# MDFahimAnjum/AliasFree-Diffusion-Models-PyTorch

Hardware: AMD Instinct MI355X
Metric: train_step_images_per_sec (higher is better)
Workload: dtype f32; 1 GPU; CIFAR-10 32x32x3 synthetic, UNet variant=3 (Config D), batch 256/GPU, T=1000, AdamW lr 3e-4, random-init weights (seed 42); global_batch=256, parallelism=dp1, hip_graph=True, launch_mode=lanes

## Files before the change

aliasfree-diffusion-models-pytorch_amd/_lib.py:

```python
import ctypes
import os
import re

_PKG = os.path.dirname(os.path.abspath(__file__))
_ROOT = os.path.dirname(_PKG)
HEADER = os.path.join(_ROOT, "include", "afd.h")
LIBPATH = os.environ.get("AFD_LIBPATH") or os.path.join(_PKG, "libafd_hip.so")

_CTYPES = {
    "int": ctypes.c_int, "long": ctypes.c_long, "float": ctypes.c_float, "double": ctypes.c_double,
    "size_t": ctypes.c_size_t,
}
_DECL = re.compile(r"^(int|size_t|const char\*)\s+(afd_\w+)\s*\(([^;]*?)\)\s*;", re.M | re.S)


def _strip_comments(src):
    return re.sub(r"/\*.*?\*/", " ", src, flags=re.S)


def parse_header(path=HEADER):
    out = {}
    for ret, name, args in _DECL.findall(_strip_comments(open(path).read())):
        argtypes = []
        args = " ".join(args.split())
        if args not in ("", "void"):
            for a in args.split(","):
                a = a.strip()
                if "*" in a or a.startswith("afd_stream_t"):
                    argtypes.append(ctypes.c_void_p)
                else:
                    base = a.split()[0] if not a.startswith("unsigned") else a
                    argtypes.append(_CTYPES[base])
        restype = {"int": ctypes.c_int, "size_t": ctypes.c_size_t, "const char*": ctypes.c_char_p}[ret]
        out[name] = (restype, argtypes)
    return out


_VALUE_RETURNING = {"afd_device_count", "afd_tok_supported", "afd_conv3x3_weight_kinds", "afd_conv_wgrad_form",
                    "afd_grad_sqnorm_n_partials"}


class AfdError(RuntimeError):
    pass


class _Lib:
    def __init__(self):
        if not os.path.exists(LIBPATH):
            raise AfdError(
                f"{LIBPATH} not found: build it with `python -c 'import __graft_entry__ as g; g.build()'` "
                "(hipcc --offload-arch=gfx950). There is no CPU/eager fallback.")
        self.cdll = ctypes.CDLL(LIBPATH)
        self.sigs = parse_header()
        for name, (restype, argtypes) in self.sigs.items():
            fn = getattr(self.cdll, name)
            fn.restype, fn.argtypes = restype, argtypes
            if restype is ctypes.c_int and name not in _VALUE_RETURNING:
                setattr(self, name, self._checked(name, fn))
            else:
                setattr(self, name, fn)

    def _checked(self, name, fn):
        last_error = self.cdll.afd_last_error
        last_error.restype = ctypes.c_char_p

        def call(*args):
            rc = fn(*args)
            if rc != 0:
                raise AfdError(f"{name} failed (code {rc}): {last_error().decode()}")
        call.__name__ = name
        return call


_lib = None


def lib():
    global _lib
    if _lib is None:
        _lib = _Lib()
    return _lib
```

aliasfree-diffusion-models-pytorch_amd/csrc/filt.hip:

```cpp
#include "common.h"

namespace afd {

__global__ void up2_fwd_gen(const float* __restrict__ x, float* __restrict__ y, int C, int H, int W,
                            long xbs, long ybs, long total, Taps t, int N) {
  const int lo = (N - 1) / 2, H2 = 2 * H, W2 = 2 * W;
  for (long i = blockIdx.x * (long)blockDim.x + threadIdx.x; i < total; i += (long)gridDim.x * blockDim.x) {
    const int q = i % W2, p = (i / W2) % H2;
    const long bc = i / ((long)W2 * H2);
    const int c = bc % C; const long b = bc / C;
    const float* xp = x + b * xbs + (long)c * H * W;
    float acc = 0.f;
    for (int a = 0; a < N; ++a) {
      const int zr = p + a - lo;
      if (zr < 0 || zr >= H2 || (zr & 1)) continue;
      for (int bb = 0; bb < N; ++bb) {
        const int zc = q + bb - lo;
        if (zc < 0 || zc >= W2 || (zc & 1)) continue;
        acc += t.k[a * N + bb] * xp[(zr >> 1) * W + (zc >> 1)];
      }
    }
    y[b * ybs + (long)c * H2 * W2 + (long)p * W2 + q] = acc;
  }
}
// ... 171 lines not shown
  xv[S] = 0.f;
  float2* yp = reinterpret_cast<float2*>(y + b * ybs + (long)c * 4 * S * S) + L.col;
  float xr = L.right(xv[0]);
#pragma unroll
  for (int i = 0; i < S; ++i) {
    const float xe = xv[i], xd = xv[i + 1];
    const float xdr = L.right(xd);
    float2 r0, r1;
    r0.x = t.k[4] * xe;
    r0.y = t.k[3] * xe + t.k[5] * xr;
    r1.x = t.k[1] * xe + t.k[7] * xd;
    r1.y = t.k[0] * xe + t.k[2] * xr + t.k[6] * xd + t.k[8] * xdr;
    if (live) { yp[(2 * i) * S] = r0; yp[(2 * i + 1) * S] = r1; }
    xr = xdr;
  }
}

template <int S, bool FULL>
__global__ __launch_bounds__(256) void down2_fwd_n3(const float* __restrict__ x, float* __restrict__ y,
                                                    long planes, int C, long xbs, long ybs, Taps3 t) {
  Lane<S> L(planes);
  if (FULL && !L.live) return;
  const bool live = FULL || L.live;
  const long b = L.plane / C; const int c = L.plane % C;
  const float2* xp = reinterpret_cast<const float2*>(x + b * xbs + (long)c * 4 * S * S) + L.col;
  float* yp = y + b * ybs + (long)c * S * S + L.col;
  float2 prev = make_float2(0.f, 0.f);
  float prev_l = 0.f;
  float2 rows[2 * S];
#pragma unroll
  for (int r = 0; r < 2 * S; ++r) rows[r] = live ? xp[r * S] : make_float2(0.f, 0.f);
#pragma unroll
  for (int i = 0; i < S; ++i) {
    const float2 mid = rows[2 * i], nxt = rows[2 * i + 1];
    const float mid_l = L.left(mid.y), nxt_l = L.left(nxt.y);
    const float d = t.k[0] * prev_l + t.k[1] * prev.x + t.k[2] * prev.y
                  + t.k[3] * mid_l  + t.k[4] * mid.x  + t.k[5] * mid.y
                  + t.k[6] * nxt_l  + t.k[7] * nxt.x  + t.k[8] * nxt.y;
    if (live) yp[i * S] = d;
    prev = nxt; prev_l = nxt_l;
  }
}

struct ActRow { float U[4], t[4]; float4 c[4]; };
struct ActG { float g00, g01, g10, g11, g01l, g11l; };

__device__ __forceinline__ void act_lookup(float U, const float4* __restrict__ T, float& t, float4& c) {
  const float sx = __builtin_amdgcn_fmed3f(fmaf(U, kGeluScale, kGeluOffset), 0.f, (float)kGeluPieces - 0.001f);
  c = T[(int)sx];
  t = __builtin_amdgcn_fractf(sx);
}
__device__ __forceinline__ float act_cubic(const float4& c, float t) { return fmaf(fmaf(fmaf(c.w, t, c.z), t, c.y), t, c.x); }

template <int S, bool FULL, bool STATS = false>
__global__ __launch_bounds__(STATS ? 1024 : 256) void filt_act_fwd_n3(const float* __restrict__ x, float* __restrict__ y,
                                                       long planes, int C, const float* __restrict__ stats,
                                                       const float* __restrict__ gamma, const float* __restrict__ beta,
                                                       const float* __restrict__ res, Taps3 u, Taps3 d,
                                                       float* __restrict__ stats_out = nullptr, float eps = 0.f) {
  __shared__ float4 T[kGeluPieces];
  load_gelu_table(T, 0, kGeluPieces);
  Lane<S> L(planes);
  const long b = L.plane / C; const int c = L.plane % C;
  const long base = L.plane * (long)S * S + L.col;
  if (FULL && !L.live) return;
  const bool live = FULL || L.live;
  float sc, sh;
  float xv[S + 2];
  if (STATS) {
    __shared__ float red[16];
#pragma unroll
    for (int i = 0; i < S; ++i) xv[i] = x[base + i * S];
    float sm = 0.f;
#pragma unroll
    for (int i = 0; i < S; ++i) sm += xv[i];
    const float n = (float)C * S * S;
    const float mean = block_sum(sm, red) / n;
    float m2 = 0.f;
#pragma unroll
    for (int i = 0; i < S; ++i) { const float dd = xv[i] - mean; m2 = fmaf(dd, dd, m2); }
    const float rstd = 1.0f / sqrtf(block_sum(m2, red) / n + eps);
    if (threadIdx.x == 0) { stats_out[2 * b] = mean; stats_out[2 * b + 1] = rstd; }
    sc = rstd * (gamma ? gamma[c] : 1.f);
    sh = (beta ? beta[c] : 0.f) - mean * sc;
#pragma unroll
    for (int i = 0; i < S; ++i) xv[i] = fmaf(xv[i], sc, sh);
  } else {
    if (live) plane_affine(stats, gamma, beta, b, c, sc, sh); else { sc = 1.f; sh = 0.f; }
#pragma unroll
    for (int i = 0; i < S; ++i) xv[i] = live ? fmaf(x[base + i * S], sc, sh) : 0.f;
  }
  if (res) {
#pragma unroll
    for (int i = 0; i < S; ++i) xv[i] += live ? res[base + i * S] : 0.f;
  }
  xv[S] = 0.f; xv[S + 1] = 0.f;
  ActRow row[2];
  ActG gg[2];
  float g10p = 0.f, g11p = 0.f, g11lp = 0.f;
  float xr0 = L.right(xv[0]), xr1 = lane_right(xv[1]);
#pragma unroll
  for (int k = 0; k < S + 2; ++k) {
    if (k < S) {
      ActRow& r = row[k & 1];
      const float xe = xv[k], xd = xv[k + 1];
      xr1 = L.right_mask(xr1);
      r.U[0] = u.k[4] * xe;
      r.U[1] = u.k[3] * xe + u.k[5] * xr0;
      r.U[2] = u.k[1] * xe + u.k[7] * xd;
      r.U[3] = u.k[0] * xe + u.k[2] * xr0 + u.k[6] * xd + u.k[8] * xr1;
#pragma unroll
      for (int q = 0; q < 4; ++q) act_lookup(r.U[q], T, r.t[q], r.c[q]);
      xr0 = xr1;
      xr1 = (k + 2 <= S) ? lane_right(xv[k + 2]) : 0.f;
    }
    __builtin_amdgcn_sched_barrier(0);
    if (k >= 2) {
      const ActG& g = gg[k & 1];
      const float g01l = L.left_mask(g.g01l), g11l = L.left_mask(g.g11l);
      const float out = d.k[0] * g11lp + d.k[1] * g10p + d.k[2] * g11p
                      + d.k[3] * g01l + d.k[4] * g.g00 + d.k[5] * g.g01
                      + d.k[6] * g11l + d.k[7] * g.g10 + d.k[8] * g.g11;
      if (live) y[base + (k - 2) * S] = out;
      g10p = g.g10; g11p = g.g11; g11lp = g11l;
    }
    __builtin_amdgcn_sched_barrier(0);
    if (k >= 1 && k <= S) {
      const ActRow& r = row[(k - 1) & 1];
      ActG& g = gg[(k - 1) & 1];
      g.g00 = r.U[0] * act_cubic(r.c[0], r.t[0]);
      g.g01 = r.U[1] * act_cubic(r.c[1], r.t[1]);
      g.g10 = r.U[2] * act_cubic(r.c[2], r.t[2]);
      g.g11 = r.U[3] * act_cubic(r.c[3], r.t[3]);
      g.g01l = lane_left(g.g01);
      g.g11l = lane_left(g.g11);
    }
    __builtin_amdgcn_sched_barrier(0);
  }
}

struct ActRowB { float t[4], dG[4]; float4 c[4]; };
struct ActGB { float dU00, dU01, dU10, dU11, dU01l, dU11l; };

template <int S, bool FULL, bool GNB = false>
__global__ __launch_bounds__(GNB ? 1024 : 256) void filt_act_bwd_n3(const float* __restrict__ x, const float* __restrict__ dy,
                                                       float* __restrict__ dv, long planes, int C,
                                                       const float* __restrict__ stats, const float* __restrict__ gamma,
                                                       const float* __restrict__ beta, const float* __restrict__ res,
                                                       float* __restrict__ part, Taps3 u, Taps3 d, float* __restrict__ dx = nullptr) {
  __shared__ float4 Tb[kGeluPieces];
  load_gelu_table(Tb, kGeluPieces, kGeluPieces);
  Lane<S> L(planes);
  const long b = L.plane / C; const int c = L.plane % C;
  const long base = L.plane * (long)S * S + L.col;
  if (FULL && !L.live) return;
  const bool live = FULL || L.live;
  float sc, sh;
  if (live) plane_affine(stats, gamma, beta, b, c, sc, sh); else { sc = 1.f; sh = 0.f; }
  float mean = 0.f, rstd = 1.f;
  if (part && live) { mean = stats[2 * b]; rstd = stats[2 * b + 1]; }
  float xv[S + 2], gv[S + 2];
  float a1 = 0.f, a2 = 0.f;
  float hx[S];
  float dvc[GNB ? S : 1];
#pragma unroll
  for (int i = 0; i < S; ++i) {
    const float h = live ? x[base + i * S] : 0.f;
    xv[i] = live ? fmaf(h, sc, sh) : 0.f;
    hx[i] = (h - mean) * rstd;
    gv[i] = live ? dy[base + i * S] : 0.f;
  }
  if (res) {
#pragma unroll
    for (int i = 0; i < S; ++i) xv[i] += live ? res[base + i * S] : 0.f;
  }
  xv[S] = 0.f; gv[S] = 0.f; xv[S + 1] = 0.f; gv[S + 1] = 0.f;
  ActRowB row[2];
  ActGB gg[2];
  float u10p = 0.f, u11p = 0.f, u11lp = 0.f;
  float xr0 = L.right(xv[0]), xr1 = lane_right(xv[1]), gr0 = L.right(gv[0]), gr1 = lane_right(gv[1]);
#pragma unroll
  for (int k = 0; k < S + 2; ++k) {
    if (k < S) {
      ActRowB& r = row[k & 1];
      const float xe = xv[k], xd = xv[k + 1], ge = gv[k], gd = gv[k + 1];
      xr1 = L.right_mask(xr1); gr1 = L.right_mask(gr1);
      const float U00 = u.k[4] * xe;
      const float U01 = u.k[3] * xe + u.k[5] * xr0;
      const float U10 = u.k[1] * xe + u.k[7] * xd;
      const float U11 = u.k[0] * xe + u.k[2] * xr0 + u.k[6] * xd + u.k[8] * xr1;
      act_lookup(U00, Tb, r.t[0], r.c[0]);
      act_lookup(U01, Tb, r.t[1], r.c[1]);
      act_lookup(U10, Tb, r.t[2], r.c[2]);
      act_lookup(U11, Tb, r.t[3], r.c[3]);
      r.dG[0] = d.k[4] * ge;
      r.dG[1] = d.k[5] * ge + d.k[3] * gr0;
      r.dG[2] = d.k[7] * ge + d.k[1] * gd;
      r.dG[3] = d.k[8] * ge + d.k[6] * gr0 + d.k[2] * gd + d.k[0] * gr1;
      xr0 = xr1; gr0 = gr1;
      xr1 = (k + 2 <= S) ? lane_right(xv[k + 2]) : 0.f;
      gr1 = (k + 2 <= S) ? lane_right(gv[k + 2]) : 0.f;
    }
    __builtin_amdgcn_sched_barrier(0);
    if (k >= 2) {
      const ActGB& g = gg[k & 1];
      const float dU01l = L.left_mask(g.dU01l), dU11l = L.left_mask(g.dU11l);
      const float out = u.k[0] * g.dU11 + u.k[1] * g.dU10 + u.k[2] * dU11l
                      + u.k[3] * g.dU01 + u.k[4] * g.dU00 + u.k[5] * dU01l
                      + u.k[6] * u11p + u.k[7] * u10p + u.k[8] * u11lp;
      if (GNB) { dvc[k - 2] = out; if (dv) dv[base + (k - 2) * S] = out; }
      else if (live) dv[base + (k - 2) * S] = out;
      a1 += out * hx[k - 2]; a2 += out;
      u10p = g.dU10; u11p = g.dU11; u11lp = dU11l;
    }
    __builtin_amdgcn_sched_barrier(0);
    if (k >= 1 && k <= S) {
      const ActRowB& r = row[(k - 1) & 1];
      ActGB& g = gg[(k - 1) & 1];
      g.dU00 = r.dG[0] * act_cubic(r.c[0], r.t[0]);
      g.dU01 = r.dG[1] * act_cubic(r.c[1], r.t[1]);
      g.dU10 = r.dG[2] * act_cubic(r.c[2], r.t[2]);
      g.dU11 = r.dG[3] * act_cubic(r.c[3], r.t[3]);
      g.dU01l = lane_left(g.dU01);
      g.dU11l = lane_left(g.dU11);
    }
    __builtin_amdgcn_sched_barrier(0);
  }
  if (GNB) {
    __shared__ float red[16];
    const float g = gamma ? gamma[c] : 1.f, n = (float)C * S * S;
    const float m1 = block_sum(g * a2, red) / n;
    const float m2 = block_sum(g * a1, red) / n;
#pragma unroll
    for (int i = 0; i < S; ++i) dx[base + i * S] = rstd * (g * dvc[i] - m1 - hx[i] * m2);
  }
  if (part) {
#pragma unroll
    for (int o = S / 2; o > 0; o >>= 1) { a1 += __shfl_xor(a1, o, kWave); a2 += __shfl_xor(a2, o, kWave); }
    if (live && L.col == 0) { part[(2 * b) * C + c] = a1; part[(2 * b + 1) * C + c] = a2; }
  }
}

static inline int gs_grid(long total, int block = 256) {
  long g = (total + block - 1) / block;
  return (int)(g < 1 ? 1 : (g > 65536 ? 65536 : g));
}
static inline bool fast_side(int H, int W) { return H == W && (H == 4 || H == 8 || H == 16 || H == 32 || H == 64); }
static inline Taps load_taps(const float* k, int N) { Taps t; for (int i = 0; i < N * N; ++i) t.k[i] = k[i]; return t; }
static inline Taps3 load_taps3(const float* k, bool rot180 = false) {
  Taps3 t; for (int i = 0; i < 9; ++i) t.k[i] = k[rot180 ? 8 - i : i]; return t;
}


#define AFD_DISPATCH_SF(S_, KERNEL, GRID_ARGS, ...)                                                      \
  if (planes % (64 / (S_)) == 0) hipLaunchKernelGGL((KERNEL<S_, true>), GRID_ARGS, __VA_ARGS__);          \
  else hipLaunchKernelGGL((KERNEL<S_, false>), GRID_ARGS, __VA_ARGS__)
#define AFD_DISPATCH_S(S_, KERNEL, GRID_ARGS, ...)                                          \
  switch (S_) {                                                                              \
    case 4:  AFD_DISPATCH_SF(4, KERNEL, GRID_ARGS, __VA_ARGS__); break;                      \
    case 8:  AFD_DISPATCH_SF(8, KERNEL, GRID_ARGS, __VA_ARGS__); break;                      \
    case 16: AFD_DISPATCH_SF(16, KERNEL, GRID_ARGS, __VA_ARGS__); break;                     \
    case 32: AFD_DISPATCH_SF(32, KERNEL, GRID_ARGS, __VA_ARGS__); break;                     \
    default: AFD_DISPATCH_SF(64, KERNEL, GRID_ARGS, __VA_ARGS__); break;                     \
  }

static inline dim3 fast_grid(long planes, int S) {
  const long ppw = 64 / S, waves = (planes + ppw - 1) / ppw;
  return dim3((unsigned)((waves + 3) / 4));
}

static int check_common(const char* fn, const void* a, const void* b, int B, int C, int H, int W, const float* taps, int N) {
  AFD_REQUIRE(a && b && taps, "%s: NULL pointer", fn);
  AFD_REQUIRE(B > 0 && C > 0 && H > 0 && W > 0, "%s: non-positive shape B=%d C=%d H=%d W=%d", fn, B, C, H, W);
  AFD_REQUIRE(N >= 1 && N <= AFD_MAX_TAPS, "%s: N=%d outside [1,%d]", fn, N, AFD_MAX_TAPS);
  return AFD_OK;
}

static int up2_like(const char* fn, const float* x, float* y, int B, int C, int H, int W, long xbs, long ybs,
                    const float* taps, int N, bool rot, hipStream_t s) {
  if (!xbs) xbs = (long)C * H * W;
  if (!ybs) ybs = (long)C * 4 * H * W;
  const long planes = (long)B * C;
  if (N == 3 && fast_side(H, W)) {
    const Taps3 t = load_taps3(taps, rot);
    AFD_DISPATCH_S(H, up2_fwd_n3, fast_grid(planes, H), dim3(256), 0, s, x, y, planes, C, xbs, ybs, t);
  } else {
    AFD_REQUIRE(!rot, "%s: internal: rot180 only on the fast path", fn);
    const long total = planes * 4 * H * W;
    hipLaunchKernelGGL(up2_fwd_gen, dim3(gs_grid(total)), dim3(256), 0, s, x, y, C, H, W, xbs, ybs, total, load_taps(taps, N), N);
  }
  return check_launch(fn);
}
// ... 40 lines not shown
  return check_launch("afd_filt_up2_bwd");
}

int afd_filt_down2_fwd(const float* x, float* y, int B, int C, int H, int W, long xbs, long ybs,
                       const float* taps, int N, afd_stream_t stream) {
  if (int e = check_common("afd_filt_down2_fwd", x, y, B, C, H, W, taps, N)) return e;
  return down2_like("afd_filt_down2_fwd", x, y, B, C, H, W, xbs, ybs, taps, N, false, as_stream(stream));
}

int afd_filt_down2_bwd(const float* dy, float* dx, int B, int C, int H, int W, long dybs, long dxbs,
                       const float* taps, int N, afd_stream_t stream) {
  if (int e = check_common("afd_filt_down2_bwd", dy, dx, B, C, H, W, taps, N)) return e;
  hipStream_t s = as_stream(stream);
  const int Ho = (H + 1) / 2, Wo = (W + 1) / 2;
  if (N == 3 && (H % 2 == 0) && (W % 2 == 0) && fast_side(Ho, Wo))
    return up2_like("afd_filt_down2_bwd", dy, dx, B, C, Ho, Wo, dybs, dxbs, taps, N, true, s);
  if (!dybs) dybs = (long)C * Ho * Wo;
  if (!dxbs) dxbs = (long)C * H * W;
  const long total = (long)B * C * H * W;
  hipLaunchKernelGGL(down2_bwd_gen, dim3(gs_grid(total)), dim3(256), 0, s, dy, dx, C, H, W, dybs, dxbs, total, load_taps(taps, N), N);
  return check_launch("afd_filt_down2_bwd");
}

size_t afd_filt_act_workspace_bytes(int B, int C, int H, int W, int N, int backward) {
  if (N == 3 && fast_side(H, W)) return 0;
  const size_t e = (size_t)B * C * H * W;
  return sizeof(float) * (backward ? 9 * e : 5 * e);
}

int afd_filt_act_fwd(const float* x, float* y, int B, int C, int H, int W,
                     const float* stats, const float* gamma, const float* beta, const float* res,
                     const float* taps_up, const float* taps_down, int N, void* workspace, afd_stream_t stream) {
  if (int e = check_common("afd_filt_act_fwd", x, y, B, C, H, W, taps_up, N)) return e;
  AFD_REQUIRE(taps_down, "afd_filt_act_fwd: taps_down is NULL");
  hipStream_t s = as_stream(stream);
  const long planes = (long)B * C;
  if (N == 3 && fast_side(H, W)) {
    const Taps3 u = load_taps3(taps_up), d = load_taps3(taps_down);
    ensure_gelu_table(s);
    AFD_DISPATCH_S(H, filt_act_fwd_n3, fast_grid(planes, H), dim3(256), 0, s, x, y, planes, C, stats, gamma, beta, res, u, d);
    return check_launch("afd_filt_act_fwd");
  }
  AFD_REQUIRE(workspace, "afd_filt_act_fwd: this shape (N=%d, %dx%d) needs a workspace", N, H, W);
  const long e = planes * H * W;
  float* v = static_cast<float*>(workspace);
  float* U = v + e;
  hipLaunchKernelGGL(prologue_gen, dim3(gs_grid(e)), dim3(256), 0, s, x, v, C, (long)H * W, e, stats, gamma, beta, res);
  hipLaunchKernelGGL(up2_fwd_gen, dim3(gs_grid(4 * e)), dim3(256), 0, s, v, U, C, H, W, (long)C * H * W, (long)C * 4 * H * W, 4 * e, load_taps(taps_up, N), N);
  hipLaunchKernelGGL(gelu_inplace_gen, dim3(gs_grid(4 * e)), dim3(256), 0, s, U, 4 * e);
  hipLaunchKernelGGL(down2_fwd_gen, dim3(gs_grid(e)), dim3(256), 0, s, U, y, C, 2 * H, 2 * W, (long)C * 4 * H * W, (long)C * H * W, e, load_taps(taps_down, N), N);
  return check_launch("afd_filt_act_fwd");
}

size_t afd_filt_act_fwd_gn_supported(int C, int H, int W, int N) {
  return (N == 3 && H == W && (H == 4 || H == 8 || H == 16) && (long)C * H <= 1024 && ((long)C * H) % 64 == 0) ? 1 : 0;
}

int afd_filt_act_fwd_gn(const float* x, float* y, int B, int C, int H, int W, float eps, float* stats_out,
                        const float* gamma, const float* beta, const float* res,
                        const float* taps_up, const float* taps_down, int N, afd_stream_t stream) {
  if (int e = check_common("afd_filt_act_fwd_gn", x, y, B, C, H, W, taps_up, N)) return e;
  AFD_REQUIRE(taps_down && stats_out, "afd_filt_act_fwd_gn: NULL pointer");
  AFD_REQUIRE(afd_filt_act_fwd_gn_supported(C, H, W, N), "afd_filt_act_fwd_gn: shape (C=%d, %dx%d, N=%d) is not covered", C, H, W, N);
  hipStream_t s = as_stream(stream);
  const Taps3 u = load_taps3(taps_up), d = load_taps3(taps_down);
  ensure_gelu_table(s);
  const long planes = (long)B * C;
  const dim3 grid((unsigned)B), block((unsigned)(C * H));
  if (H == 4) hipLaunchKernelGGL((filt_act_fwd_n3<4, true, true>), grid, block, 0, s, x, y, planes, C, nullptr, gamma, beta, res, u, d, stats_out, eps);
  else if (H == 8) hipLaunchKernelGGL((filt_act_fwd_n3<8, true, true>), grid, block, 0, s, x, y, planes, C, nullptr, gamma, beta, res, u, d, stats_out, eps);
  else hipLaunchKernelGGL((filt_act_fwd_n3<16, true, true>), grid, block, 0, s, x, y, planes, C, nullptr, gamma, beta, res, u, d, stats_out, eps);
  return check_launch("afd_filt_act_fwd_gn");
}

int afd_filt_act_bwd_gn(const float* x, const float* dy, float* dx, float* dres, int B, int C, int H, int W, const float* stats,
                        const float* gamma, const float* beta, const float* res, const float* taps_up, const float* taps_down, int N,
                        float* gn_partials, afd_stream_t stream) {
  if (int e = check_common("afd_filt_act_bwd_gn", x, dy, B, C, H, W, taps_up, N)) return e;
  AFD_REQUIRE(dx && taps_down && stats && gn_partials, "afd_filt_act_bwd_gn: NULL pointer");
  AFD_REQUIRE(afd_filt_act_fwd_gn_supported(C, H, W, N), "afd_filt_act_bwd_gn: shape (C=%d, %dx%d, N=%d) is not covered", C, H, W, N);
  hipStream_t s = as_stream(stream);
  const Taps3 u = load_taps3(taps_up), d = load_taps3(taps_down);
  ensure_gelu_table(s);
  const long planes = (long)B * C;
  const dim3 grid((unsigned)B), block((unsigned)(C * H));
  if (H == 4) hipLaunchKernelGGL((filt_act_bwd_n3<4, true, true>), grid, block, 0, s, x, dy, dres, planes, C, stats, gamma, beta, res, gn_partials, u, d, dx);
  else if (H == 8) hipLaunchKernelGGL((filt_act_bwd_n3<8, true, true>), grid, block, 0, s, x, dy, dres, planes, C, stats, gamma, beta, res, gn_partials, u, d, dx);
  else hipLaunchKernelGGL((filt_act_bwd_n3<16, true, true>), grid, block, 0, s, x, dy, dres, planes, C, stats, gamma, beta, res, gn_partials, u, d, dx);
  return check_launch("afd_filt_act_bwd_gn");
}

int afd_filt_act_bwd(const float* x, const float* dy, float* dv, int B, int C, int H, int W,
                     const float* stats, const float* gamma, const float* beta, const float* res,
                     const float* taps_up, const float* taps_down, int N, void* workspace, float* gn_partials,
                     afd_stream_t stream) {
  if (int e = check_common("afd_filt_act_bwd", x, dy, B, C, H, W, taps_up, N)) return e;
  AFD_REQUIRE(dv && taps_down, "afd_filt_act_bwd: NULL pointer");
  hipStream_t s = as_stream(stream);
  const long planes = (long)B * C;
  if (N == 3 && fast_side(H, W)) {
    const Taps3 u = load_taps3(taps_up), d = load_taps3(taps_down);
    AFD_REQUIRE(!gn_partials || stats, "afd_filt_act_bwd: gn_partials needs stats");
    ensure_gelu_table(s);
    AFD_DISPATCH_S(H, filt_act_bwd_n3, fast_grid(planes, H), dim3(256), 0, s, x, dy, dv, planes, C, stats, gamma, beta, res, gn_partials, u, d);
    return check_launch("afd_filt_act_bwd");
  }
  AFD_REQUIRE(workspace, "afd_filt_act_bwd: this shape (N=%d, %dx%d) needs a workspace", N, H, W);
  AFD_REQUIRE(!gn_partials, "afd_filt_act_bwd: gn_partials are produced on the fused fast path only (workspace_bytes == 0)");
  const long e = planes * H * W;
  float* v = static_cast<float*>(workspace);
  float* U = v + e;
  float* dG = U + 4 * e;
  const long cs = (long)C * H * W, cs4 = 4 * cs;
  hipLaunchKernelGGL(prologue_gen, dim3(gs_grid(e)), dim3(256), 0, s, x, v, C, (long)H * W, e, stats, gamma, beta, res);
  hipLaunchKernelGGL(up2_fwd_gen, dim3(gs_grid(4 * e)), dim3(256), 0, s, v, U, C, H, W, cs, cs4, 4 * e, load_taps(taps_up, N), N);
  hipLaunchKernelGGL(down2_bwd_gen, dim3(gs_grid(4 * e)), dim3(256), 0, s, dy, dG, C, 2 * H, 2 * W, cs, cs4, 4 * e, load_taps(taps_down, N), N);
  hipLaunchKernelGGL(gelu_grad_mul_gen, dim3(gs_grid(4 * e)), dim3(256), 0, s, U, dG, 4 * e);
  hipLaunchKernelGGL(up2_bwd_gen, dim3(gs_grid(e)), dim3(256), 0, s, dG, dv, C, H, W, cs4, cs, e, load_taps(taps_up, N), N);
  return check_launch("afd_filt_act_bwd");
}

}
```

aliasfree-diffusion-models-pytorch_amd/ops.py:

```python
import weakref

import numpy as np
import os
import torch

from ._lib import AfdError, lib

GN_EPS = 1e-5
LN_EPS = 1e-5
NULL_LABEL = -1


_raw_stream = getattr(torch._C, "_cuda_getCurrentRawStream", None)
_get_device = getattr(torch._C, "_cuda_getDevice", None) or torch.cuda.current_device


def _stream():
    if _raw_stream is not None:
        return _raw_stream(_get_device())
    return torch.cuda.current_stream().cuda_stream


def _chk(*tensors):
    for t in tensors:
# ... 255 lines not shown
    return out[0], out[1], 0, (out[0], out[1])


class GroupNorm1(_Fn):

    @staticmethod
    def forward(ctx, x, gamma, beta, res, emb, act):
        _chk(x, gamma, beta, res, emb)
        x, res, emb = _c(x), _c(res), _c(emb)
        B, C, H, W = x.shape
        y = torch.empty_like(x)
        stats = torch.empty(B, 2, device=x.device, dtype=torch.float32)
        lib().afd_groupnorm1_fwd(_p(x), _p(y), _p(stats), B, C, H * W, GN_EPS, _p(gamma), _p(beta), _p(res), act,
                                 _p(emb), _stream())
        ctx.save_for_backward(x, gamma, beta, res, stats)
        ctx.act, ctx.has_emb = act, emb is not None
        return y

    @staticmethod
    def backward(ctx, dy):
        x, gamma, beta, res, stats = ctx.saved_tensors
        B, C, H, W = x.shape
        dy = _c(dy)
        dx = torch.empty_like(x)
        dres = None
        if res is not None:
            dres = dy if ctx.act == 0 else torch.empty_like(x)
        part = torch.empty(B * C * 2, device=x.device, dtype=torch.float32)
        demb = torch.empty(B, C, device=x.device, dtype=torch.float32) if ctx.has_emb else None
        dg, db, acc, (dgamma, dbeta) = _gn_param_targets(C, gamma, beta, x.device)
        defer = acc and _GradMode.side is not None
        lib().afd_groupnorm1_bwd(_p(x), _p(dy), _p(stats), B, C, H * W, _p(gamma), _p(beta), _p(res), ctx.act,
                                 _p(dx), _p(dres) if (res is not None and ctx.act == 1) else None, _p(part), _p(demb), 0,
                                 None if defer else _p(dg), None if defer else _p(db), acc, _stream())
        if defer:
            pp = _p(part)
            defer_to_side_stream(None, fold_desc(pp, _p(dg), C, B, stride=2 * C) + fold_desc(pp + 4 * C, _p(db), C, B, stride=2 * C),
                                 part, writes=(gamma, beta))
        elif acc:
            _wrote(gamma, beta)
        return dx, dgamma, dbeta, dres, demb, None


class GroupNormFiltAct(_Fn):

    @staticmethod
    def forward(ctx, x, gamma, beta, res, tu, td):
        _chk(x, gamma, beta, res)
        x, res = _c(x), _c(res)
        B, C, H, W = x.shape
        stats = torch.empty(B, 2, device=x.device, dtype=torch.float32)
        L = lib()
        y = torch.empty_like(x)
        if L.afd_filt_act_fwd_gn_supported(C, H, W, tu.N):
            L.afd_filt_act_fwd_gn(_p(x), _p(y), B, C, H, W, GN_EPS, _p(stats), _p(gamma), _p(beta), _p(res), tu.ptr, td.ptr, tu.N,
                                  _stream())
        else:
            L.afd_groupnorm1_fwd(_p(x), None, _p(stats), B, C, H * W, GN_EPS, None, None, None, 0, None, _stream())
            ws = _act_ws(B, C, H, W, tu.N, 0, x.device)
            L.afd_filt_act_fwd(_p(x), _p(y), B, C, H, W, _p(stats), _p(gamma), _p(beta), _p(res), tu.ptr, td.ptr, tu.N,
                               _p(ws), _stream())
        ctx.save_for_backward(x, gamma, beta, res, stats)
        ctx.tu, ctx.td = tu, td
        return y

    @staticmethod
    def backward(ctx, dy):
        x, gamma, beta, res, stats = ctx.saved_tensors
        B, C, H, W = x.shape
        dy = _c(dy)
        L = lib()
        if L.afd_filt_act_fwd_gn_supported(C, H, W, ctx.tu.N):
            dx = torch.empty_like(x)
            dres = torch.empty_like(x) if res is not None else None
            part = torch.empty(B * C * 2, device=x.device, dtype=torch.float32)
            L.afd_filt_act_bwd_gn(_p(x), _p(dy), _p(dx), _p(dres), B, C, H, W, _p(stats), _p(gamma), _p(beta), _p(res),
                                  ctx.tu.ptr, ctx.td.ptr, ctx.tu.N, _p(part), _stream())
            dg, db, acc, (dgamma, dbeta) = _gn_param_targets(C, gamma, beta, x.device)
            if acc and _GradMode.side is not None:
                pp = _p(part)
                defer_to_side_stream(None, fold_desc(pp, _p(dg), C, B, stride=2 * C) + fold_desc(pp + 4 * C, _p(db), C, B, stride=2 * C),
                                     part, writes=(gamma, beta))
            else:
                L.afd_colsum2(_p(part), _p(dg), _p(db), B, C, acc, _stream())
                if acc:
                    _wrote(gamma, beta)
            return dx, dgamma, dbeta, dres, None, None
        dv = torch.empty_like(x)
        ws = _act_ws(B, C, H, W, ctx.tu.N, 1, x.device)
        part = torch.empty(B * C * 2, device=x.device, dtype=torch.float32)
        fused = ws is None
        L.afd_filt_act_bwd(_p(x), _p(dy), _p(dv), B, C, H, W, _p(stats), _p(gamma), _p(beta), _p(res),
                           ctx.tu.ptr, ctx.td.ptr, ctx.tu.N, _p(ws), _p(part) if fused else None, _stream())
        dx = torch.empty_like(x)
        dg, db, acc, (dgamma, dbeta) = _gn_param_targets(C, gamma, beta, x.device)
        L.afd_groupnorm1_bwd(_p(x), _p(dv), _p(stats), B, C, H * W, _p(gamma), _p(beta), None, 0,
                             _p(dx), None, _p(part), None, 1 if fused else 0, _p(dg), _p(db), acc, _stream())
        if acc:
            _wrote(gamma, beta)
        return dx, dgamma, dbeta, (dv if res is not None else None), None, None


def _kind_of(kinds, dgrad):
    direct = kinds >> dgrad & 1
    return direct | (kinds & 4 if direct else 0)


class _WinoWeights:
    epoch = 0
    store = {}
    max_entries = 4096
    recording = None
    active_plan = None

    @classmethod
    def get(cls, w, nbytes, dgrad, kinds=0):
        plan = cls.active_plan
        if plan is not None:
            u = plan.lookup(w, nbytes, dgrad, kinds)
            if u is not None:
                return u, 1
        if cls.recording is not None:
            rec = cls.recording.setdefault(id(w), [w, 0, 0, 0])
            rec[1 + dgrad] = nbytes
            rec[3] = kinds
# ... 1662 lines not shown
```

include/afd.h:

```cpp
#ifndef AFD_H_
#define AFD_H_

#include <stddef.h>
#include <stdint.h>

#ifdef __cplusplus
extern "C" {
#endif

#define AFD_OK 0
#define AFD_EINVAL 1
#define AFD_ELAUNCH 2
#define AFD_MAX_TAPS 15

typedef void* afd_stream_t;

const char* afd_version(void);
const char* afd_last_error(void);
int afd_device_count(void);

int afd_lowpass_kernel(double omega_c, int N, int has_beta, double beta, float* taps_out);

int afd_filt_up2_fwd(const float* x, float* y, int B, int C, int H, int W, long x_bstride, long y_bstride,
                     const float* taps, int N, afd_stream_t stream);
int afd_filt_up2_bwd(const float* dy, float* dx, int B, int C, int H, int W, long dy_bstride, long dx_bstride,
                     const float* taps, int N, afd_stream_t stream);

int afd_filt_down2_fwd(const float* x, float* y, int B, int C, int H, int W, long x_bstride, long y_bstride,
                       const float* taps, int N, afd_stream_t stream);
int afd_filt_down2_bwd(const float* dy, float* dx, int B, int C, int H, int W, long dy_bstride, long dx_bstride,
                       const float* taps, int N, afd_stream_t stream);

size_t afd_filt_act_workspace_bytes(int B, int C, int H, int W, int N, int backward);
int afd_filt_act_fwd(const float* x, float* y, int B, int C, int H, int W,
                     const float* stats, const float* gamma, const float* beta, const float* res,
                     const float* taps_up, const float* taps_down, int N,
                     void* workspace, afd_stream_t stream);
size_t afd_filt_act_fwd_gn_supported(int C, int H, int W, int N);
int afd_filt_act_fwd_gn(const float* x, float* y, int B, int C, int H, int W, float eps, float* stats_out,
                        const float* gamma, const float* beta, const float* res,
                        const float* taps_up, const float* taps_down, int N, afd_stream_t stream);
int afd_filt_act_bwd_gn(const float* x, const float* dy, float* dx, float* dres, int B, int C, int H, int W, const float* stats,
                        const float* gamma, const float* beta, const float* res, const float* taps_up, const float* taps_down, int N,
                        float* gn_partials, afd_stream_t stream);
int afd_filt_act_bwd(const float* x, const float* dy, float* dv, int B, int C, int H, int W,
                     const float* stats, const float* gamma, const float* beta, const float* res,
                     const float* taps_up, const float* taps_down, int N,
                     void* workspace, float* gn_partials, afd_stream_t stream);

int afd_groupnorm1_fwd(const float* x, float* y, float* stats_out, int B, int C, int HW, float eps,
                       const float* gamma, const float* beta, const float* res, int act, const float* emb,
                       afd_stream_t stream);
int afd_debug_norm_path(int mode);
int afd_groupnorm1_bwd(const float* x, const float* dy, const float* stats, int B, int C, int HW,
                       const float* gamma, const float* beta, const float* res, int act,
                       float* dx, float* dres, float* dgamma_dbeta_partial , float* demb ,
                       int have_partials ,
                       float* dgamma , float* dbeta , int accumulate, afd_stream_t stream);
int afd_colsum(const float* in, float* out, int rows, int cols, int accumulate, afd_stream_t stream);
int afd_colsum_strided(const float* in, long row_stride, float* out, int rows, int cols, int accumulate, afd_stream_t stream);
int afd_colsum2(const float* in, float* out_a, float* out_b, int rows, int C, int accumulate, afd_stream_t stream);

int afd_debug_conv_path(int mode);
int afd_conv_fwd(const float* x, const float* w, const float* bias, const float* res, float* y,
                 int B, int Cin, int Cout, int H, int W, int ksize, int act, afd_stream_t stream);
int afd_conv_dgrad(const float* dy, const float* w, float* dx,
                   int B, int Cin, int Cout, int H, int W, int ksize, afd_stream_t stream);
size_t afd_conv_wgrad_workspace_bytes(int B, int Cin, int Cout, int H, int W, int ksize);
int afd_conv_wgrad_form(int B, int Cin, int Cout, int H, int W, int ksize);
int afd_conv_wgrad(const float* x, const float* dy, float* dw, float* dbias ,
                   int B, int Cin, int Cout, int H, int W, int ksize, int accumulate,
                   void* workspace, afd_stream_t stream);

typedef struct afd_fold_desc {
  const float* part;
  float* dst;
  long n;
  long stride;
  long inner, rstride;
  int splits;
  int accumulate;
} afd_fold_desc;
int afd_fold_batched(const afd_fold_desc* descs, int n, afd_stream_t stream);
int afd_conv_wgrad_partials(const float* x, const float* dy, float* dw, float* dbias ,
                            int B, int Cin, int Cout, int H, int W, int ksize, int accumulate,
                            void* workspace, afd_fold_desc* folds_out, int* n_folds, afd_stream_t stream);

size_t afd_conv3x3_wino_workspace_bytes(int B, int Cin, int Cout, int H, int W, int dgrad);
int afd_conv3x3_wino_weights(const float* w, float* u_fwd, float* u_dgrad, int Cin, int Cout, int kinds, afd_stream_t stream);
int afd_conv3x3_weight_kinds(int B, int Cin, int Cout, int H, int W);
typedef struct afd_wino_desc {
// ... 316 lines not shown
```

Measured before the change: 37160 images/s.

## Extend sample-resident fused GroupNorm+filtered-activation kernels to 32x32 and C*H=2048 shapes

Widens the one-block-per-sample fused GroupNorm+up/act/down kernels to cover 32x32 planes and shapes with C*H=2048. For the larger case each lane handles two planes, and the backward pass parks dv in dynamic LDS, then recomputes normalized x in a second pass to finish the GN backward inside the kernel. The aim is to drop the separate stats/partials passes and their extra global round-trips on high-resolution layers. A CU-count heuristic picks this path only when the batch gives enough blocks. Large LDS use and heavier per-thread register load may cut occupancy.

```diff
diff --git a/aliasfree-diffusion-models-pytorch_amd/_lib.py b/aliasfree-diffusion-models-pytorch_amd/_lib.py
--- a/aliasfree-diffusion-models-pytorch_amd/_lib.py
+++ b/aliasfree-diffusion-models-pytorch_amd/_lib.py
@@ -37,7 +37,7 @@
 
 
 _VALUE_RETURNING = {"afd_device_count", "afd_tok_supported", "afd_conv3x3_weight_kinds", "afd_conv_wgrad_form",
-                    "afd_grad_sqnorm_n_partials"}
+                    "afd_grad_sqnorm_n_partials", "afd_filt_act_gn_resident"}
 
 
 class AfdError(RuntimeError):
diff --git a/aliasfree-diffusion-models-pytorch_amd/csrc/filt.hip b/aliasfree-diffusion-models-pytorch_amd/csrc/filt.hip
--- a/aliasfree-diffusion-models-pytorch_amd/csrc/filt.hip
+++ b/aliasfree-diffusion-models-pytorch_amd/csrc/filt.hip
@@ -247,44 +247,65 @@
 }
 __device__ __forceinline__ float act_cubic(const float4& c, float t) { return fmaf(fmaf(fmaf(c.w, t, c.z), t, c.y), t, c.x); }
 
-template <int S, bool FULL, bool STATS = false>
+template <int S, bool FULL, bool STATS = false, int NP = 1>
 __global__ __launch_bounds__(STATS ? 1024 : 256) void filt_act_fwd_n3(const float* __restrict__ x, float* __restrict__ y,
                                                        long planes, int C, const float* __restrict__ stats,
                                                        const float* __restrict__ gamma, const float* __restrict__ beta,
                                                        const float* __restrict__ res, Taps3 u, Taps3 d,
                                                        float* __restrict__ stats_out = nullptr, float eps = 0.f) {
+  static_assert(NP == 1 || STATS, "two planes per lane: sample-resident form only");
   __shared__ float4 T[kGeluPieces];
   load_gelu_table(T, 0, kGeluPieces);
   Lane<S> L(planes);
-  const long b = L.plane / C; const int c = L.plane % C;
-  const long base = L.plane * (long)S * S + L.col;
   if (FULL && !L.live) return;
   const bool live = FULL || L.live;
-  float sc, sh;
-  float xv[S + 2];
+  float xvv[NP][S + 2];
+  float scv[NP], shv[NP];
+  long basev[NP];
+#pragma unroll
+  for (int pp = 0; pp < NP; ++pp) {
+    const long plane = NP == 1 ? L.plane : (long)blockIdx.x * C + threadIdx.x / S + pp * (C / NP);
+    basev[pp] = plane * (long)S * S + L.col;
+  }
   if (STATS) {
     __shared__ float red[16];
-#pragma unroll
-    for (int i = 0; i < S; ++i) xv[i] = x[base + i * S];
+    const long b = blockIdx.x;
+#pragma unroll
+    for (int pp = 0; pp < NP; ++pp)
+#pragma unroll
+      for (int i = 0; i < S; ++i) xvv[pp][i] = x[basev[pp] + i * S];
     float sm = 0.f;
 #pragma unroll
-    for (int i = 0; i < S; ++i) sm += xv[i];
+    for (int pp = 0; pp < NP; ++pp)
+#pragma unroll
+      for (int i = 0; i < S; ++i) sm += xvv[pp][i];
     const float n = (float)C * S * S;
     const float mean = block_sum(sm, red) / n;
     float m2 = 0.f;
 #pragma unroll
-    for (int i = 0; i < S; ++i) { const float dd = xv[i] - mean; m2 = fmaf(dd, dd, m2); }
+    for (int pp = 0; pp < NP; ++pp)
+#pragma unroll
+      for (int i = 0; i < S; ++i) { const float dd = xvv[pp][i] - mean; m2 = fmaf(dd, dd, m2); }
     const float rstd = 1.0f / sqrtf(block_sum(m2, red) / n + eps);
     if (threadIdx.x == 0) { stats_out[2 * b] = mean; stats_out[2 * b + 1] = rstd; }
-    sc = rstd * (gamma ? gamma[c] : 1.f);
-    sh = (beta ? beta[c] : 0.f) - mean * sc;
-#pragma unroll
-    for (int i = 0; i < S; ++i) xv[i] = fmaf(xv[i], sc, sh);
+#pragma unroll
+    for (int pp = 0; pp < NP; ++pp) {
+      const int c = NP == 1 ? (int)(L.plane % C) : (int)(threadIdx.x / S) + pp * (C / NP);
+      scv[pp] = rstd * (gamma ? gamma[c] : 1.f);
+      shv[pp] = (beta ? beta[c] : 0.f) - mean * scv[pp];
+#pragma unroll
+      for (int i = 0; i < S; ++i) xvv[pp][i] = fmaf(xvv[pp][i], scv[pp], shv[pp]);
+    }
   } else {
-    if (live) plane_affine(stats, gamma, beta, b, c, sc, sh); else { sc = 1.f; sh = 0.f; }
-#pragma unroll
-    for (int i = 0; i < S; ++i) xv[i] = live ? fmaf(x[base + i * S], sc, sh) : 0.f;
-  }
+    const long b = L.plane / C; const int c = L.plane % C;
+    if (live) plane_affine(stats, gamma, beta, b, c, scv[0], shv[0]); else { scv[0] = 1.f; shv[0] = 0.f; }
+#pragma unroll
+    for (int i = 0; i < S; ++i) xvv[0][i] = live ? fmaf(x[basev[0] + i * S], scv[0], shv[0]) : 0.f;
+  }
+#pragma unroll
+  for (int pp = 0; pp < NP; ++pp) {
+  float (&xv)[S + 2] = xvv[pp];
+  const long base = basev[pp];
   if (res) {
 #pragma unroll
     for (int i = 0; i < S; ++i) xv[i] += live ? res[base + i * S] : 0.f;
@@ -332,38 +353,49 @@
     }
     __builtin_amdgcn_sched_barrier(0);
   }
+  }
 }
 
 struct ActRowB { float t[4], dG[4]; float4 c[4]; };
 struct ActGB { float dU00, dU01, dU10, dU11, dU01l, dU11l; };
 
-template <int S, bool FULL, bool GNB = false>
+template <int S, bool FULL, int GNB = 0, int NP = 1>
 __global__ __launch_bounds__(GNB ? 1024 : 256) void filt_act_bwd_n3(const float* __restrict__ x, const float* __restrict__ dy,
                                                        float* __restrict__ dv, long planes, int C,
                                                        const float* __restrict__ stats, const float* __restrict__ gamma,
                                                        const float* __restrict__ beta, const float* __restrict__ res,
                                                        float* __restrict__ part, Taps3 u, Taps3 d, float* __restrict__ dx = nullptr) {
+  static_assert(NP == 1 || GNB == 2, "two planes per lane: LDS-parked sample-resident form only");
   __shared__ float4 Tb[kGeluPieces];
+  extern __shared__ float dvl[];
   load_gelu_table(Tb, kGeluPieces, kGeluPieces);
   Lane<S> L(planes);
-  const long b = L.plane / C; const int c = L.plane % C;
-  const long base = L.plane * (long)S * S + L.col;
   if (FULL && !L.live) return;
   const bool live = FULL || L.live;
+  const long b = NP == 1 ? L.plane / C : (long)blockIdx.x;
+  float mean = 0.f, rstd = 1.f;
+  if (part && live) { mean = stats[2 * b]; rstd = stats[2 * b + 1]; }
+  float a1v[NP], a2v[NP];
+  int cv[NP];
+  long basev[NP];
+  float hx[S];
+  float dvc[GNB == 1 ? S : 1];
+  constexpr int kPF = S / 4;
+#pragma unroll
+  for (int pp = 0; pp < NP; ++pp) {
+  const int c = NP == 1 ? (int)(L.plane % C) : (int)(threadIdx.x / S) + pp * (C / NP);
+  const long base = (NP == 1 ? L.plane : b * C + c) * (long)S * S + L.col;
+  cv[pp] = c; basev[pp] = base;
   float sc, sh;
   if (live) plane_affine(stats, gamma, beta, b, c, sc, sh); else { sc = 1.f; sh = 0.f; }
-  float mean = 0.f, rstd = 1.f;
-  if (part && live) { mean = stats[2 * b]; rstd = stats[2 * b + 1]; }
   float xv[S + 2], gv[S + 2];
   float a1 = 0.f, a2 = 0.f;
-  float hx[S];
-  float dvc[GNB ? S : 1];
 #pragma unroll
   for (int i = 0; i < S; ++i) {
     const float h = live ? x[base + i * S] : 0.f;
     xv[i] = live ? fmaf(h, sc, sh) : 0.f;
-    hx[i] = (h - mean) * rstd;
-    gv[i] = live ? dy[base + i * S] : 0.f;
+    if (GNB != 2) hx[i] = (h - mean) * rstd;
+    if (GNB != 2 || i < kPF + 2) gv[i] = live ? dy[base + i * S] : 0.f;
   }
   if (res) {
 #pragma unroll
@@ -378,6 +410,7 @@
   for (int k = 0; k < S + 2; ++k) {
     if (k < S) {
       ActRowB& r = row[k & 1];
+      if (GNB == 2 && k + 2 + kPF < S) gv[k + 2 + kPF] = dy[base + (k + 2 + kPF) * S];
       const float xe = xv[k], xd = xv[k + 1], ge = gv[k], gd = gv[k + 1];
       xr1 = L.right_mask(xr1); gr1 = L.right_mask(gr1);
       const float U00 = u.k[4] * xe;
@@ -403,9 +436,11 @@
       const float out = u.k[0] * g.dU11 + u.k[1] * g.dU10 + u.k[2] * dU11l
                       + u.k[3] * g.dU01 + u.k[4] * g.dU00 + u.k[5] * dU01l
                       + u.k[6] * u11p + u.k[7] * u10p + u.k[8] * u11lp;
-      if (GNB) { dvc[k - 2] = out; if (dv) dv[base + (k - 2) * S] = out; }
+      if (GNB == 1) { dvc[k - 2] = out; if (dv) dv[base + (k - 2) * S] = out; }
+      else if (GNB == 2) { dvl[(pp * S + k - 2) * blockDim.x + threadIdx.x] = out; if (dv) dv[base + (k - 2) * S] = out; }
       else if (live) dv[base + (k - 2) * S] = out;
-      a1 += out * hx[k - 2]; a2 += out;
+      if (GNB != 2) a1 += out * hx[k - 2];
+      a2 += out;
       u10p = g.dU10; u11p = g.dU11; u11lp = dU11l;
     }
     __builtin_amdgcn_sched_barrier(0);
@@ -421,18 +456,49 @@
     }
     __builtin_amdgcn_sched_barrier(0);
   }
-  if (GNB) {
+  a1v[pp] = a1; a2v[pp] = a2;
+  }
+  if (GNB == 1) {
     __shared__ float red[16];
-    const float g = gamma ? gamma[c] : 1.f, n = (float)C * S * S;
-    const float m1 = block_sum(g * a2, red) / n;
-    const float m2 = block_sum(g * a1, red) / n;
-#pragma unroll
-    for (int i = 0; i < S; ++i) dx[base + i * S] = rstd * (g * dvc[i] - m1 - hx[i] * m2);
+    const float g = gamma ? gamma[cv[0]] : 1.f, n = (float)C * S * S;
+    const float m1 = block_sum(g * a2v[0], red) / n;
+    const float m2 = block_sum(g * a1v[0], red) / n;
+#pragma unroll
+    for (int i = 0; i < S; ++i) dx[basev[0] + i * S] = rstd * (g * dvc[i] - m1 - hx[i] * m2);
+  }
+  if (GNB == 2) {
+    __shared__ float red[16];
+    const float n = (float)C * S * S;
+    asm volatile("" ::: "memory");
+    float gm[NP], xh[NP][S], dvr[NP][S], s1 = 0.f, s2 = 0.f;
+#pragma unroll
+    for (int pp = 0; pp < NP; ++pp) {
+      gm[pp] = gamma ? gamma[cv[pp]] : 1.f;
+      float a1 = 0.f;
+#pragma unroll
+      for (int i = 0; i < S; ++i) {
+        xh[pp][i] = (x[basev[pp] + i * S] - mean) * rstd;
+        dvr[pp][i] = dvl[(pp * S + i) * blockDim.x + threadIdx.x];
+        a1 += dvr[pp][i] * xh[pp][i];
+      }
+      a1v[pp] = a1;
+      s1 += gm[pp] * a2v[pp]; s2 += gm[pp] * a1;
+    }
+    const float m1 = block_sum(s1, red) / n;
+    const float m2 = block_sum(s2, red) / n;
+#pragma unroll
+    for (int pp = 0; pp < NP; ++pp)
+#pragma unroll
+      for (int i = 0; i < S; ++i) dx[basev[pp] + i * S] = rstd * (gm[pp] * dvr[pp][i] - m1 - xh[pp][i] * m2);
   }
   if (part) {
 #pragma unroll
-    for (int o = S / 2; o > 0; o >>= 1) { a1 += __shfl_xor(a1, o, kWave); a2 += __shfl_xor(a2, o, kWave); }
-    if (live && L.col == 0) { part[(2 * b) * C + c] = a1; part[(2 * b + 1) * C + c] = a2; }
+    for (int pp = 0; pp < NP; ++pp) {
+      float a1 = a1v[pp], a2 = a2v[pp];
+#pragma unroll
+      for (int o = S / 2; o > 0; o >>= 1) { a1 += __shfl_xor(a1, o, kWave); a2 += __shfl_xor(a2, o, kWave); }
+      if (live && L.col == 0) { part[(2 * b) * C + cv[pp]] = a1; part[(2 * b + 1) * C + cv[pp]] = a2; }
+    }
   }
 }
 
@@ -579,8 +645,37 @@
   return check_launch("afd_filt_act_fwd");
 }
 
-size_t afd_filt_act_fwd_gn_supported(int C, int H, int W, int N) {
-  return (N == 3 && H == W && (H == 4 || H == 8 || H == 16) && (long)C * H <= 1024 && ((long)C * H) % 64 == 0) ? 1 : 0;
+static int gn_form(int C, int H, int W, int N) {
+  if (N != 3 || H != W) return 0;
+  const long t = (long)C * H;
+  if ((H == 4 || H == 8 || H == 16) && t <= 1024 && t % 64 == 0) return 1;
+  if (H == 32 && t <= 1024 && t % 64 == 0) return 2;
+  if ((H == 8 || H == 16) && t == 2048) return 2;
+  return 0;
+}
+static int g_act_path = 0;
+static int device_cus() {
+  static int cus[64] = {0};
+  int dev = 0;
+  if (hipGetDevice(&dev) != hipSuccess || dev < 0 || dev >= 64) return 0;
+  if (!cus[dev]) {
+    int n = 0;
+    if (hipDeviceGetAttribute(&n, hipDeviceAttributeMultiprocessorCount, dev) != hipSuccess) return 0;
+    cus[dev] = n;
+  }
+  return cus[dev];
+}
+
+int afd_debug_filt_act_path(int mode) { g_act_path = (mode == 1 || mode == 2) ? mode : 0; return AFD_OK; }
+
+size_t afd_filt_act_fwd_gn_supported(int C, int H, int W, int N) { return gn_form(C, H, W, N) ? 1 : 0; }
+
+int afd_filt_act_gn_resident(int B, int C, int H, int W, int N) {
+  const int form = gn_form(C, H, W, N);
+  if (!form || g_act_path == 1 || B < 1) return 0;
+  if (form == 1 || g_act_path == 2) return 1;
+  const int cus = device_cus();
+  return cus > 0 && 2L * B >= cus ? 1 : 0;
 }
 
 int afd_filt_act_fwd_gn(const float* x, float* y, int B, int C, int H, int W, float eps, float* stats_out,
@@ -588,16 +683,32 @@
                         const float* taps_up, const float* taps_down, int N, afd_stream_t stream) {
   if (int e = check_common("afd_filt_act_fwd_gn", x, y, B, C, H, W, taps_up, N)) return e;
   AFD_REQUIRE(taps_down && stats_out, "afd_filt_act_fwd_gn: NULL pointer");
-  AFD_REQUIRE(afd_filt_act_fwd_gn_supported(C, H, W, N), "afd_filt_act_fwd_gn: shape (C=%d, %dx%d, N=%d) is not covered", C, H, W, N);
+  const int form = gn_form(C, H, W, N);
+  AFD_REQUIRE(form, "afd_filt_act_fwd_gn: shape (C=%d, %dx%d, N=%d) is not covered", C, H, W, N);
   hipStream_t s = as_stream(stream);
   const Taps3 u = load_taps3(taps_up), d = load_taps3(taps_down);
   ensure_gelu_table(s);
   const long planes = (long)B * C;
-  const dim3 grid((unsigned)B), block((unsigned)(C * H));
-  if (H == 4) hipLaunchKernelGGL((filt_act_fwd_n3<4, true, true>), grid, block, 0, s, x, y, planes, C, nullptr, gamma, beta, res, u, d, stats_out, eps);
-  else if (H == 8) hipLaunchKernelGGL((filt_act_fwd_n3<8, true, true>), grid, block, 0, s, x, y, planes, C, nullptr, gamma, beta, res, u, d, stats_out, eps);
-  else hipLaunchKernelGGL((filt_act_fwd_n3<16, true, true>), grid, block, 0, s, x, y, planes, C, nullptr, gamma, beta, res, u, d, stats_out, eps);
+  const int np = (long)C * H > 1024 ? 2 : 1;
+  const dim3 grid((unsigned)B), block((unsigned)(C * H / np));
+#define AFD_FWD_GN(S_, NP_) hipLaunchKernelGGL((filt_act_fwd_n3<S_, true, true, NP_>), grid, block, 0, s, x, y, planes, C, nullptr, gamma, beta, res, u, d, stats_out, eps)
+  if (np == 2) { if (H == 8) AFD_FWD_GN(8, 2); else AFD_FWD_GN(16, 2); }
+  else if (H == 4) AFD_FWD_GN(4, 1);
+  else if (H == 8) AFD_FWD_GN(8, 1);
+  else if (H == 16) AFD_FWD_GN(16, 1);
+  else AFD_FWD_GN(32, 1);
+#undef AFD_FWD_GN
   return check_launch("afd_filt_act_fwd_gn");
+}
+
+extern "C++" template <int S, int NP>
+static int launch_bwd_gn_lds(hipStream_t s, int B, int C, const float* x, const float* dy, float* dres, const float* stats, const float* gamma,
+                             const float* beta, const float* res, float* part, const Taps3& u, const Taps3& d, float* dx) {
+  const size_t lds = sizeof(float) * (size_t)C * S * S;
+  if (int rc = lds_opt_in(filt_act_bwd_n3<S, true, 2, NP>, lds)) return rc;
+  hipLaunchKernelGGL((filt_act_bwd_n3<S, true, 2, NP>), dim3((unsigned)B), dim3((unsigned)(C * S / NP)), lds, s, x, dy, dres, (long)B * C, C,
+                     stats, gamma, beta, res, part, u, d, dx);
+  return AFD_OK;
 }
 
 int afd_filt_act_bwd_gn(const float* x, const float* dy, float* dx, float* dres, int B, int C, int H, int W, const float* stats,
@@ -605,15 +716,23 @@
                         float* gn_partials, afd_stream_t stream) {
   if (int e = check_common("afd_filt_act_bwd_gn", x, dy, B, C, H, W, taps_up, N)) return e;
   AFD_REQUIRE(dx && taps_down && stats && gn_partials, "afd_filt_act_bwd_gn: NULL pointer");
-  AFD_REQUIRE(afd_filt_act_fwd_gn_supported(C, H, W, N), "afd_filt_act_bwd_gn: shape (C=%d, %dx%d, N=%d) is not covered", C, H, W, N);
+  const int form = gn_form(C, H, W, N);
+  AFD_REQUIRE(form, "afd_filt_act_bwd_gn: shape (C=%d, %dx%d, N=%d) is not covered", C, H, W, N);
   hipStream_t s = as_stream(stream);
   const Taps3 u = load_taps3(taps_up), d = load_taps3(taps_down);
   ensure_gelu_table(s);
   const long planes = (long)B * C;
+  if (form == 2) {
+    int rc;
+    if (H == 32) rc = launch_bwd_gn_lds<32, 1>(s, B, C, x, dy, dres, stats, gamma, beta, res, gn_partials, u, d, dx);
+    else if (H == 16) rc = launch_bwd_gn_lds<16, 2>(s, B, C, x, dy, dres, stats, gamma, beta, res, gn_partials, u, d, dx);
+    else rc = launch_bwd_gn_lds<8, 2>(s, B, C, x, dy, dres, stats, gamma, beta, res, gn_partials, u, d, dx);
+    return rc ? rc : check_launch("afd_filt_act_bwd_gn");
+  }
   const dim3 grid((unsigned)B), block((unsigned)(C * H));
-  if (H == 4) hipLaunchKernelGGL((filt_act_bwd_n3<4, true, true>), grid, block, 0, s, x, dy, dres, planes, C, stats, gamma, beta, res, gn_partials, u, d, dx);
-  else if (H == 8) hipLaunchKernelGGL((filt_act_bwd_n3<8, true, true>), grid, block, 0, s, x, dy, dres, planes, C, stats, gamma, beta, res, gn_partials, u, d, dx);
-  else hipLaunchKernelGGL((filt_act_bwd_n3<16, true, true>), grid, block, 0, s, x, dy, dres, planes, C, stats, gamma, beta, res, gn_partials, u, d, dx);
+  if (H == 4) hipLaunchKernelGGL((filt_act_bwd_n3<4, true, 1>), grid, block, 0, s, x, dy, dres, planes, C, stats, gamma, beta, res, gn_partials, u, d, dx);
+  else if (H == 8) hipLaunchKernelGGL((filt_act_bwd_n3<8, true, 1>), grid, block, 0, s, x, dy, dres, planes, C, stats, gamma, beta, res, gn_partials, u, d, dx);
+  else hipLaunchKernelGGL((filt_act_bwd_n3<16, true, 1>), grid, block, 0, s, x, dy, dres, planes, C, stats, gamma, beta, res, gn_partials, u, d, dx);
   return check_launch("afd_filt_act_bwd_gn");
 }
 
diff --git a/aliasfree-diffusion-models-pytorch_amd/ops.py b/aliasfree-diffusion-models-pytorch_amd/ops.py
--- a/aliasfree-diffusion-models-pytorch_amd/ops.py
+++ b/aliasfree-diffusion-models-pytorch_amd/ops.py
@@ -331,7 +331,8 @@
         stats = torch.empty(B, 2, device=x.device, dtype=torch.float32)
         L = lib()
         y = torch.empty_like(x)
-        if L.afd_filt_act_fwd_gn_supported(C, H, W, tu.N):
+        resident = bool(L.afd_filt_act_gn_resident(B, C, H, W, tu.N))
+        if resident:
             L.afd_filt_act_fwd_gn(_p(x), _p(y), B, C, H, W, GN_EPS, _p(stats), _p(gamma), _p(beta), _p(res), tu.ptr, td.ptr, tu.N,
                                   _stream())
         else:
@@ -340,7 +341,7 @@
             L.afd_filt_act_fwd(_p(x), _p(y), B, C, H, W, _p(stats), _p(gamma), _p(beta), _p(res), tu.ptr, td.ptr, tu.N,
                                _p(ws), _stream())
         ctx.save_for_backward(x, gamma, beta, res, stats)
-        ctx.tu, ctx.td = tu, td
+        ctx.tu, ctx.td, ctx.resident = tu, td, resident
         return y
 
     @staticmethod
@@ -349,7 +350,7 @@
         B, C, H, W = x.shape
         dy = _c(dy)
         L = lib()
-        if L.afd_filt_act_fwd_gn_supported(C, H, W, ctx.tu.N):
+        if ctx.resident:
             dx = torch.empty_like(x)
             dres = torch.empty_like(x) if res is not None else None
             part = torch.empty(B * C * 2, device=x.device, dtype=torch.float32)
diff --git a/include/afd.h b/include/afd.h
--- a/include/afd.h
+++ b/include/afd.h
@@ -37,6 +37,8 @@
                      const float* taps_up, const float* taps_down, int N,
                      void* workspace, afd_stream_t stream);
 size_t afd_filt_act_fwd_gn_supported(int C, int H, int W, int N);
+int afd_filt_act_gn_resident(int B, int C, int H, int W, int N);
+int afd_debug_filt_act_path(int mode);
 int afd_filt_act_fwd_gn(const float* x, float* y, int B, int C, int H, int W, float eps, float* stats_out,
                         const float* gamma, const float* beta, const float* res,
                         const float* taps_up, const float* taps_down, int N, afd_stream_t stream);
```

Result: no change. 37520 images/s, median of 6 (+1.0%).
